# maropu/hivemall

Measured on AMD Instinct MI355X. Metric: rows/sec (node) FFM on Criteo-shaped sparse at 1/2/4/8 MI355X; logloss parity, higher is better.
Workload: dtype fp32; 1 GPU; global_batch=262144, seq_len=39, nnz_per_row=39, fields=explicit, parallelism=dp1, mix_every=10, state=fp32 V, fp32 AdaGrad accumulator per (feature, field) slot (fp32 math), state_layout=packed, reload=False, mixed_bytes_per_mix=671088656, mix_overlapped=False, mix_wire=bf16_delta, early_ramp_warmup_steps=1, linear_steps=side-table, resident_batches=8

## Files before the change

csrc/kernels/ffm.hip:

```cpp
#include <type_traits>

#include "common.h"

namespace {

struct FFMParams {
    int B, F;
    int num_features, num_fields, Kp;
    int classification;
    int train;
    int use_linear, use_bias, norm;
    int reload;
    int gstride;
    int vpad;
    int tail16;
    int gfstride;
    int sstride;
    int fstride;
    long long vfe;
    uint32_t seed;
    float eta0, eps, lambda_v;
    float alpha, beta, lambda1, lambda2;
    float min_target, max_target;
    const void* reserved;
    int32_t* defer;
    int list_mode;
    int lin_defer;
    long long lstride;
    int lpack;
    int lin_atomic;
    const int32_t* hidx;
    const int32_t* hot_id;
    float* hacc;
    int nhot;
    int hacc_on;
    float* bias_sh;
    int bias_s;
    int bias_every;
};

#define LW(p, i) ((p)[(size_t)(i) * (size_t)P.lstride])

__device__ __forceinline__ float ftrl_weight(float z, float n, float alpha, float beta,
                                             float l1, float l2) {
    if (fabsf(z) <= l1) return 0.f;
    const float s = z > 0.f ? 1.f : -1.f;
    return -(z - s * l1) / ((beta + sqrtf(n)) / alpha + l2);
}

__device__ __forceinline__ float ftrl_update(float* __restrict__ z, float* __restrict__ n,
                                             float w, float g, float alpha, float beta,
                                             float l1, float l2) {
    const float n0 = *n;
    const float n1 = n0 + g * g;
    const float sigma = (sqrtf(n1) - sqrtf(n0)) / alpha;
    const float z1 = *z + g - sigma * w;
    *z = z1;
    *n = n1;
    return ftrl_weight(z1, n1, alpha, beta, l1, l2);
}

__device__ __forceinline__ float bias_w0(const FFMParams& P, const float* bias) {
    const float z = __hip_atomic_load(bias + 1, __ATOMIC_RELAXED, __HIP_MEMORY_SCOPE_AGENT);
    const float n = __hip_atomic_load(bias + 2, __ATOMIC_RELAXED, __HIP_MEMORY_SCOPE_AGENT);
    return ftrl_weight(z, n, P.alpha, P.beta, 0.f, 0.f);
}

__device__ __forceinline__ void bias_update(const FFMParams& P, float g, float* bias) {
    const float z0 = __hip_atomic_load(bias + 1, __ATOMIC_RELAXED, __HIP_MEMORY_SCOPE_AGENT);
    const float n0 = __hip_atomic_load(bias + 2, __ATOMIC_RELAXED, __HIP_MEMORY_SCOPE_AGENT);
    const float w = ftrl_weight(z0, n0, P.alpha, P.beta, 0.f, 0.f);
    const float sigma = (sqrtf(n0 + g * g) - sqrtf(n0)) / P.alpha;
    const float dz = g - sigma * w;
    atomicAdd(bias + 1, dz);
    atomicAdd(bias + 2, g * g);
    bias[0] = ftrl_weight(z0 + dz, n0 + g * g, P.alpha, P.beta, 0.f, 0.f);
}

__device__ __forceinline__ void bias_update_sh(const FFMParams& P, float g, float z0, float n0, float* sh,
                                               float* acc) {
    const float w = ftrl_weight(z0, n0, P.alpha, P.beta, 0.f, 0.f);
    const float sigma = (sqrtf(n0 + g * g) - sqrtf(n0)) / P.alpha;
    const float dz = g - sigma * w;
    atomicAdd(sh, dz);
    atomicAdd(sh + 1, g * g);
    acc[0] += dz;
    acc[1] += g * g;
}

constexpr int HD_SIZE = 2048;
constexpr int HD12_SIZE = 1024;
constexpr int HACC_READ_STRIDE = 4;
__host__ __device__ __forceinline__ int hacc_read_off(int nhot) { return (2 * nhot + 31) & ~31; }

template <int TPB>
__device__ __forceinline__ void hacc_publish(float* __restrict__ hacc, int nhot, int tid) {
    typedef float f4v __attribute__((ext_vector_type(4)));
    float4* rd = reinterpret_cast<float4*>(hacc + hacc_read_off(nhot));
    for (int t = 2 * tid; t < nhot; t += 2 * TPB) {
        const f4v a = __builtin_nontemporal_load(reinterpret_cast<const f4v*>(hacc) + (t >> 1));
        rd[(HACC_READ_STRIDE / 4) * t] = make_float4(a.x, a.y, 0.f, 0.f);
        if (t + 1 < nhot) rd[(HACC_READ_STRIDE / 4) * (t + 1)] = make_float4(a.z, a.w, 0.f, 0.f);
    }
}
constexpr int HACC_GRID = 2048;
constexpr int HACC_GRID12 = 2304;

__device__ __forceinline__ uint32_t hash3(uint32_t a, uint32_t b, uint32_t c) {
    uint32_t h = a * 0x9E3779B1u ^ (b + 0x7F4A7C15u) * 0x85EBCA77u ^ c * 0xC2B2AE3Du;
    h ^= h >> 15; h *= 0x2C1B3C6Du; h ^= h >> 12; h *= 0x297A2D39u; h ^= h >> 15;
    return h;
}

template <bool BF>
__device__ __forceinline__ float4 ld_chunk(const void* base, size_t off) {
    if constexpr (BF) {
        const uint2 q = *reinterpret_cast<const uint2*>(reinterpret_cast<const uint16_t*>(base) + off);
        return make_float4(__uint_as_float(q.x << 16), __uint_as_float(q.x & 0xFFFF0000u),
                           __uint_as_float(q.y << 16), __uint_as_float(q.y & 0xFFFF0000u));
    } else {
        return *reinterpret_cast<const float4*>(reinterpret_cast<const float*>(base) + off);
    }
}

template <bool BF>
__device__ __forceinline__ typename std::conditional<BF, uint2, float4>::type ld_raw(const void* base, size_t off) {
    if constexpr (BF) return *reinterpret_cast<const uint2*>(reinterpret_cast<const uint16_t*>(base) + off);
    else return *reinterpret_cast<const float4*>(reinterpret_cast<const float*>(base) + off);
}

template <bool BF, typename T>
__device__ __forceinline__ float4 to_f4(const T& q) {
    if constexpr (BF) {
        return make_float4(__uint_as_float(q.x << 16), __uint_as_float(q.x & 0xFFFF0000u),
                           __uint_as_float(q.y << 16), __uint_as_float(q.y & 0xFFFF0000u));
    } else {
        return q;
    }
}

template <bool BF>
__device__ __forceinline__ void st_chunk(void* base, size_t off, float4 v, uint32_t rnd) {
    if constexpr (BF) {
        const uint32_t r2 = rnd * 0x9E3779B1u + 0x632BE5ABu;
        const uint32_t lo = hm::pack_bf16x2_sr(v.x, rnd, v.y, rnd >> 16);
        const uint32_t hi = hm::pack_bf16x2_sr(v.z, r2, v.w, r2 >> 16);
        *reinterpret_cast<uint2*>(reinterpret_cast<uint16_t*>(base) + off) = make_uint2(lo, hi);
    } else {
        *reinterpret_cast<float4*>(reinterpret_cast<float*>(base) + off) = v;
    }
}

struct SlotMeta {
    int i, f;
    float x;
};

__device__ __forceinline__ SlotMeta fetch_row_meta(const FFMParams& P, int row,
                                                   const int32_t* __restrict__ idx,
                                                   const int32_t* __restrict__ fld,
                                                   const float* __restrict__ val) {
    SlotMeta m{-1, 0, 0.f};
    const int tid = threadIdx.x;
    if (tid < P.F && row < P.B) {
        const size_t o = (size_t)row * P.F + tid;
        m.i = idx[o];
        m.f = fld ? fld[o] : tid;
        m.x = val ? val[o] : 1.f;
    }
    return m;
}

__device__ __forceinline__ float publish_row_meta(const FFMParams& P, SlotMeta m, int* s_idx,
                                                  int* s_fld, float* s_x, float* s_red) {
    const int tid = threadIdx.x;
    float sq = 0.f;
// ... 599 lines not shown
                o0 = o0 + meta * d0 * r0;
                o1 = o1 + meta * d1 * r1;
                const uint32_t h = rotl32(hrow, 5 * j + 1) ^ (0x9E3779B9u * (uint32_t)(j + 1));
                const uint4 st = make_uint4(pack_sr_hi(o0, h, rotl32(h, 16)),
                                            pack_sr_hi(o1, rotl32(h, 8), rotl32(h, 24)),
                                            pack_sr_hi(g0, rotl32(h, 4), rotl32(h, 20)),
                                            pack_sr_hi(g1, rotl32(h, 12), rotl32(h, 28)));
                if (wr >> j & 1u) *reinterpret_cast<uint4*>(vg + off[j]) = st;
            }
            if (wave == 0 && lane < F) {
                const int pi = s_m[cur][lane].x;
                if (pi >= 0) {
                    for (int f = P.num_fields; f < (int)nfld; ++f)
                        *reinterpret_cast<uint4*>(vg + ((uint32_t)pi * nfld + (uint32_t)f) * SLOT_B) = make_uint4(0u, 0u, 0u, 0u);
                }
            }
            if (mi >= 0) {
                if (P.use_linear) {
                    const float lz = s_lin[cur][1][lane];
                    const float ln = s_lin[cur][2][lane];
                    const float g = kappa * mx * scale;
                    const float n1 = ln + g * g;
                    const float z1 = lz + g - (sqrtf(n1) - sqrtf(ln)) / P.alpha * lw;
                    LW(wz, mi) = z1;
                    LW(wn, mi) = n1;
                    LW(w, mi) = ftrl_weight(z1, n1, P.alpha, P.beta, P.lambda1, P.lambda2);
                }
            }
            if (P.use_bias && tid == 0) bias_update(P, kappa, bias);
        }
        if (more) dma_lin(nxt);
    }
    __builtin_amdgcn_s_waitcnt(0x0F70);
#undef SA
#undef SB
}


typedef uint32_t u3v_t __attribute__((ext_vector_type(3)));

#define VMCNT_ENC(n) ((((n) & 15) | (((n) >> 4) << 14)) | 0x0F70)
template <bool PIN>
__device__ __forceinline__ float dot4_products_rounded(float4 c, float4 p) {
    float m0 = c.x * p.x, m1 = c.y * p.y, m2 = c.z * p.z, m3 = c.w * p.w;
    if constexpr (PIN) asm("" : "+v"(m0), "+v"(m1), "+v"(m2), "+v"(m3));
    return m0 + m1 + m2 + m3;
}

constexpr int SG32_TRAIN = 1;

template <int NS, typename OT, int TPB = 256, int ATOM = 0, int KV = 1, int KEEP = 0, int LT = 0, int CFG = 0>
__global__ __launch_bounds__(TPB) __attribute__((amdgpu_waves_per_eu(TPB / 128))) void ffm_pipe_sg32_kernel(
    FFMParams P, const int32_t* __restrict__ idx, const int32_t* __restrict__ fld,
    const float* __restrict__ val, const float* __restrict__ y, void* __restrict__ Vt,
    float* __restrict__ Gt, float* __restrict__ w, float* __restrict__ wz, float* __restrict__ wn,
    float* __restrict__ bias, float* __restrict__ pred_out, float* __restrict__ loss_out)
{
    constexpr bool SPEC = (CFG & SG32_TRAIN) != 0;
    static_assert(!SPEC || (ATOM == 0 && KV == 1 && KEEP >= 2 && sizeof(OT) == 4 && TPB % 64 == 0 &&
                            TPB >= 256 && NS <= 8 && NS * TPB < (1 << 15)),
                  "SG32_TRAIN: the default fp32 k <= 4 training launch only");
#define c_train (SPEC || P.train)
#define c_linear (SPEC || P.use_linear)
#define c_lpack (SPEC || P.lpack)
#define c_ldefer (SPEC || P.lin_defer)
#define c_bias (!SPEC && P.use_bias)
#define c_fld (SPEC || fld)
#define c_val (SPEC || val)
#define c_hacc (SPEC ? LT != 0 : P.hacc_on)
    __shared__ __attribute__((aligned(16))) float4 s_rv[NS * TPB * KV];
    __shared__ __attribute__((aligned(16))) float s_rg[NS * TPB];
    __shared__ __attribute__((aligned(16))) float4 s_t[NS * TPB * KV];
    __shared__ __attribute__((aligned(16))) int4 s_m[2][48];
    __shared__ __attribute__((aligned(16))) int s_mr[2][3][48];
    __shared__ __attribute__((aligned(16))) float s_lin[2][3][48];
    __shared__ __attribute__((aligned(16))) float4 s_lin4[2][48];
    __shared__ float s_red[TPB / 64 + 2];
    __shared__ int s_rep[TPB / 64];
    __shared__ float s_bias[4];
    __shared__ float s_bcur[2];
    __shared__ float2 s_hd[LT ? HD_SIZE : 1];
    __shared__ __attribute__((aligned(16))) float4 s_hacc[LT ? 2 : 1][48];
    __shared__ __attribute__((aligned(16))) int s_nh[LT ? 2 : 1][48];
    const int F = P.F;
    const int FF = F * F;
    const int tid = threadIdx.x, lane = tid & 63;
    const int wave = SPEC ? __builtin_amdgcn_readfirstlane(tid >> 6) : tid >> 6;
    constexpr int W_META = 1, W_LIN = 2, W_DMA = 3;
    const OT vfs = (OT)P.fstride * (16u * KV);
    const OT gfs = (OT)P.gstride * 4u;
    const int G = (int)gridDim.x;
    const int bid = (int)blockIdx.x;
    char* vb = reinterpret_cast<char*>(Vt);
    char* gb = reinterpret_cast<char*>(Gt);
    if constexpr (LT != 0) {
        for (int t = tid; t < HD_SIZE; t += TPB) s_hd[t] = make_float2(0.f, 0.f);
    }
    int nh = -1, kh = -1;
    const float* hread = LT ? P.hacc + hacc_read_off(P.nhot) : nullptr;

    int ab[NS];
    uint32_t okm = 0u;
#pragma unroll
    for (int j = 0; j < NS; ++j) {
        const int s = tid + j * TPB;
        if constexpr (SPEC) {
            const int a = s < FF ? s / F : 0, b = s < FF ? s % F : 0;
            ab[j] = (a << 4) | (b << 10) | ((s < FF ? b * F + a : s) << 16);
            okm |= (uint32_t)(s >= FF) << j | (uint32_t)(s >= FF || a == b) << (8 + j) | (uint32_t)(a < b) << (16 + j);
        } else {
            ab[j] = s < FF ? (s / F) | ((s % F) << 8) : 0;
        }
    }
#define SA(j) (SPEC ? (ab[j] >> 4) & 0x3F : ab[j] & 0xFF)
#define SB(j) (SPEC ? (ab[j] >> 10) & 0x3F : ab[j] >> 8)
#define ST(j) (SPEC ? ab[j] >> 16 : (SB(j) * F + SA(j)) * KV)

    auto dma_meta = [&](int bf, int row) {
        if (wave == W_DMA && lane < F && row < P.B) {
            const size_t o = (size_t)row * F + lane;
            __builtin_amdgcn_global_load_lds((glb_ptr_t)(idx + o), (lds_ptr_t)&s_mr[bf][0][0], 4, 0, 0);
            if (c_fld) __builtin_amdgcn_global_load_lds((glb_ptr_t)(fld + o), (lds_ptr_t)&s_mr[bf][1][0], 4, 0, 0);
            if (c_val) __builtin_amdgcn_global_load_lds((glb_ptr_t)(val + o), (lds_ptr_t)&s_mr[bf][2][0], 4, 0, 0);
        }
    };
    auto publish_meta = [&](int bf) {
        if (wave == W_META) {
            float sq = 0.f;
            if (lane < F) {
                int ri = s_mr[bf][0][lane];
                int rf = c_fld ? s_mr[bf][1][lane] : lane;
                float rx = c_val ? __int_as_float(s_mr[bf][2][lane]) : 1.f;
                if (ri < 0 || ri >= P.num_features || rf < 0 || rf >= P.num_fields) { ri = -1; rx = 0.f; rf = 0; }
                const int hb = SPEC && ri >= 0 ? (int)((uint32_t)ri * (uint32_t)vfs) : 0;
                s_m[bf][lane] = make_int4(ri, rf, __float_as_int(rx), hb);
                sq = rx * rx;
            }
            const float tot = hm::wave_sum_uniform(sq);
            if (lane == 0) s_red[TPB / 64 + bf] = (P.norm && tot > 0.f) ? rsqrtf(tot) : 1.f;
        }
    };
    auto slot = [&](int bf, int j, OT& ov, OT& og, float& xab) -> uint32_t {
        const int4 ma = s_m[bf][SA(j)], mb = s_m[bf][SB(j)];
        const bool ok = (ma.x | mb.x) >= 0 && tid + j * TPB < FF;
        const bool live = ok && SA(j) != SB(j);
        const OT i = ok ? (OT)(uint32_t)ma.x : (OT)0, f = ok ? (OT)(uint32_t)mb.y : (OT)0;
        ov = i * vfs + f * (16u * KV);
        og = i * gfs + f * 4u;
        xab = live ? __int_as_float(ma.z) * __int_as_float(mb.z) : 0.f;
        return live ? 1u : (ok ? 2u : 0u);
    };
    OT kov[KEEP ? NS : 1], kog[KEEP ? NS : 1], nov[KEEP ? NS : 1], nog[KEEP ? NS : 1];
    float kxab[KEEP ? NS : 1], nxab[KEEP ? NS : 1];
    uint32_t klive = 0u, kwr = 0u, nlive = 0u, nwr = 0u;
    int krep = 0, nrep = 0;
    auto dma_slots = [&](int bf) {
        if constexpr (KEEP) { nlive = 0u; nwr = 0u; nrep = 0; }
        if constexpr (SPEC) {
            uint32_t eq = 0u;
#pragma unroll
            for (int j = 0; j < NS; ++j) {
                const int4 ma = s_m[bf][SA(j)], mb = s_m[bf][SB(j)];
                const int both = ma.x | mb.x;
                const bool ok = (both | (int)(okm << (31 - j))) >= 0;
                const bool live = (both | (int)(okm << (23 - j))) >= 0;
                const OT ib = ok ? (OT)(uint32_t)ma.w : (OT)0, f = ok ? (OT)(uint32_t)mb.y : (OT)0;
                OT f4 = f * 4u;
                asm("" : "+v"(f4));
                nov[j] = ib + f * 16u;
                nog[j] = ib + f4;
                nxab[j] = live ? __int_as_float(ma.z) * __int_as_float(mb.z) : 0.f;
                nwr |= (uint32_t)ok << j;
                eq |= (uint32_t)(ma.x == mb.x || ma.y == mb.y) << j;
                __builtin_amdgcn_global_load_lds((glb_ptr_t)(vb + nov[j]), (lds_ptr_t)(s_rv + j * TPB + wave * 64), 16, 0, 0);
                __builtin_amdgcn_global_load_lds((glb_ptr_t)(gb + nog[j]), (lds_ptr_t)(s_rg + j * TPB + wave * 64), 4, 0, 0);
            }
            nlive = nwr & ~(okm >> 8);
            if (P.defer) nrep = (int)(eq & nwr & (okm >> 16));
            return;
        }
#pragma unroll
        for (int j = 0; j < NS; ++j) {
            OT ov, og;
            float xab;
            const uint32_t k = slot(bf, j, ov, og, xab);
            if constexpr (KEEP) {
                nov[j] = ov;
                nog[j] = og;
                nxab[j] = xab;
                nlive |= (k & 1u) << j;
                nwr |= (uint32_t)(k != 0u) << j;
                if (P.defer) nrep |= (int)slot_repeats(SA(j), SB(j), s_m[bf][SA(j)], s_m[bf][SB(j)]);
            }
#pragma unroll
            for (int q = 0; q < KV; ++q)
                __builtin_amdgcn_global_load_lds((glb_ptr_t)(vb + ov + 16u * q),
                                                 (lds_ptr_t)(s_rv + (q * NS + j) * TPB + wave * 64), 16, 0, 0);
            __builtin_amdgcn_global_load_lds((glb_ptr_t)(gb + og), (lds_ptr_t)(s_rg + j * TPB + wave * 64), 4, 0, 0);
        }
    };
    auto keep_rotate = [&]() {
        if constexpr (KEEP) {
#pragma unroll
            for (int j = 0; j < NS; ++j) { kov[j] = nov[j]; kog[j] = nog[j]; kxab[j] = nxab[j]; }
            klive = nlive; kwr = nwr; krep = nrep;
        }
    };
    const int nlin = (c_linear && c_ldefer) ? ((c_lpack || !c_train) ? 1 + (LT != 0) : 3) : 0;
    auto dma_lin = [&](int bf) {
        if (c_linear && wave == W_LIN && lane < F) {
            const int i = max(s_m[bf][lane].x, 0);
            if (c_lpack) {
                __builtin_amdgcn_global_load_lds((glb_ptr_t)&LW(w, i), (lds_ptr_t)&s_lin4[bf][0], 16, 0, 0);
                if constexpr (LT != 0)
                    __builtin_amdgcn_global_load_lds((glb_ptr_t)(hread + HACC_READ_STRIDE * max(nh, 0)), (lds_ptr_t)&s_hacc[bf][0], 16, 0, 0);
                return;
            }
            __builtin_amdgcn_global_load_lds((glb_ptr_t)&LW(w, i), (lds_ptr_t)&s_lin[bf][0][0], 4, 0, 0);
            if (c_train) {
                __builtin_amdgcn_global_load_lds((glb_ptr_t)&LW(wz, i), (lds_ptr_t)&s_lin[bf][1][0], 4, 0, 0);
                __builtin_amdgcn_global_load_lds((glb_ptr_t)&LW(wn, i), (lds_ptr_t)&s_lin[bf][2][0], 4, 0, 0);
            }
        }
    };

    int row = bid;
    if (row >= P.B) return;
    if (tid == 0) { s_bcur[0] = 0.f; s_bcur[1] = 0.f; }
    dma_meta(0, row);
    if constexpr (LT != 0) {
        if (c_hacc) hacc_publish<TPB>(P.hacc, P.nhot, tid);
    }
    __builtin_amdgcn_s_waitcnt(0x0F70);
    bar_raw();
    publish_meta(0);
    bar_raw();
    dma_slots(0);
    keep_rotate();
    if constexpr (LT != 0) {
        if (wave == W_LIN && lane < F) nh = s_m[0][lane].x >= 0 ? P.hidx[s_m[0][lane].x] : -1;
    }
    dma_lin(0);
    kh = nh;
    dma_meta(1, row + G);

    float4 fv[NS][KV];
    float fg[NS];
    OT fo[NS];
    uint32_t fwd = 0u;
    const bool bsh = c_bias && P.bias_sh;
    int bit = 0;
    float bz = 0.f, bn = 0.f;
    if (bsh && wave == W_META && lane < P.bias_s) {
        bz = __hip_atomic_load(P.bias_sh + lane * 32, __ATOMIC_RELAXED, __HIP_MEMORY_SCOPE_AGENT);
        bn = __hip_atomic_load(P.bias_sh + lane * 32 + 1, __ATOMIC_RELAXED, __HIP_MEMORY_SCOPE_AGENT);
    }
    for (int cur = 0; row < P.B; row += G, cur ^= 1) {
        const int nxt = cur ^ 1;
        const bool more = row + G < P.B;
        if constexpr (SPEC) asm volatile("" : "+v"(okm));
        if (wave == W_LIN && nlin == 3) __builtin_amdgcn_s_waitcnt(0x0F73);
        else if (wave == W_LIN && nlin == 2) __builtin_amdgcn_s_waitcnt(0x0F72);
        else if (wave == W_LIN && nlin == 1) __builtin_amdgcn_s_waitcnt(0x0F71);
        else __builtin_amdgcn_s_waitcnt(0x0F70);
        bar_raw();
        const bool bre = bsh && bit > 0 && (bit % P.bias_every) == 0;
        float nbz = bz, nbn = bn;
        if (bre && wave == W_META && lane < P.bias_s) {
            nbz = __hip_atomic_load(P.bias_sh + lane * 32, __ATOMIC_RELAXED, __HIP_MEMORY_SCOPE_AGENT);
            nbn = __hip_atomic_load(P.bias_sh + lane * 32 + 1, __ATOMIC_RELAXED, __HIP_MEMORY_SCOPE_AGENT);
        }
        if constexpr (LT != 0) {
            if (more && wave == W_LIN && lane < F) {
                const int ri = s_mr[nxt][0][lane];
                __builtin_amdgcn_global_load_lds((glb_ptr_t)(P.hidx + (ri >= 0 && ri < P.num_features ? ri : 0)),
                                                 (lds_ptr_t)&s_nh[nxt][0], 4, 0, 0);
            }
        }
        float cg[NS];
        float4 own[SPEC ? NS : 1];
#pragma unroll
        for (int j = 0; j < NS; ++j) {
            cg[j] = s_rg[j * TPB + tid];
            float4 v[KV];
#pragma unroll
            for (int q = 0; q < KV; ++q) v[q] = s_rv[(q * NS + j) * TPB + tid];
            if (fwd >> j & 1u) {
                bool same;
                if constexpr (KEEP) {
                    same = (kwr >> j & 1u) && kov[j] == fo[j];
                } else {
                    OT ov, og;
                    float xq;
                    same = slot(cur, j, ov, og, xq) != 0u && ov == fo[j];
                }
                if (same) {
#pragma unroll
                    for (int q = 0; q < KV; ++q) v[q] = fv[j][q];
                    cg[j] = fg[j];
                }
            }
            if constexpr (SPEC) {
                s_t[ST(j)] = v[0];
                own[j] = v[0];
            } else if (tid + j * TPB < FF) {
#pragma unroll
                for (int q = 0; q < KV; ++q) s_t[ST(j) + q] = v[q];
            }
        }
        fwd = 0u;
        if (more) publish_meta(nxt);
        bar_raw();
        if (more) {
            dma_slots(nxt);
            dma_meta(cur, row + 2 * G);
        }
        const float scale = s_red[TPB / 64 + cur];
        int mi = -1;
// ... 91 lines not shown
                float gs = cg[j];
#pragma unroll
                for (int q = 0; q < KV; ++q) {
                    const float4 pv = KEEP >= 2 ? kpv[j][q] : s_t[s * KV + q];
                    const float4 cv = KEEP >= 2 ? kcv[j][q] : s_t[ST(j) + q];
                    o0[q] = f2{cv.x, cv.y};
                    o1[q] = f2{cv.z, cv.w};
                    const f2 p0 = f2{pv.x, pv.y}, p1 = f2{pv.z, pv.w};
                    d0[q] = cc * p0 + ll * o0[q];
                    d1[q] = cc * p1 + ll * o1[q];
                    gs = (((gs + d0[q].x * d0[q].x) + d0[q].y * d0[q].y) + d1[q].x * d1[q].x) + d1[q].y * d1[q].y;
                }
                const float r = __builtin_amdgcn_rsqf(gs + P.eps) * -P.eta0;
                const f2 rr = {r, r};
#pragma unroll
                for (int q = 0; q < KV; ++q) {
                    const f2 n0 = o0[q] + rr * d0[q], n1 = o1[q] + rr * d1[q];
                    fv[j][q] = make_float4(n0.x, n0.y, n1.x, n1.y);
                }
                fg[j] = gs;
                fo[j] = ov;
                fwd |= 1u << j;
                if (ATOM == 1) {
                    if (live >> j & 1u) {
                        float* vp = reinterpret_cast<float*>(vb + ov);
#pragma unroll
                        for (int q = 0; q < KV; ++q) {
                            const f2 e0 = rr * d0[q], e1 = rr * d1[q];
                            atomicAdd(vp + 4 * q + 0, e0.x);
                            atomicAdd(vp + 4 * q + 1, e0.y);
                            atomicAdd(vp + 4 * q + 2, e1.x);
                            atomicAdd(vp + 4 * q + 3, e1.y);
                        }
                        atomicAdd(reinterpret_cast<float*>(gb + og), gs - cg[j]);
                    }
                    continue;
                }
#pragma unroll
                for (int q = 0; q < KV; ++q) *reinterpret_cast<float4*>(vb + ov + 16u * q) = fv[j][q];
                *reinterpret_cast<float*>(gb + og) = fg[j];
            }
            if (mi >= 0) {
                if (c_linear) {
                    const float lz = hot ? hz : (c_lpack ? s_lin4[cur][lane].y : s_lin[cur][1][lane]);
                    const float ln = hot ? hn : (c_lpack ? s_lin4[cur][lane].z : s_lin[cur][2][lane]);
                    const float g = kappa * mx * scale;
                    const float n1 = ln + g * g;
                    const float z1 = lz + g - (sqrtf(n1) - sqrtf(ln)) / P.alpha * lw;
                    const float w1 = ftrl_weight(z1, n1, P.alpha, P.beta, P.lambda1, P.lambda2);
                    if (LT && hot) {
                        const float2 d = s_hd[kh];
                        s_hd[kh] = make_float2(d.x + (g - (sqrtf(n1) - sqrtf(ln)) / P.alpha * lw), d.y + g * g);
                    } else if (ATOM == 1) {
                        atomicAdd(&LW(wz, mi), z1 - lz);
                        atomicAdd(&LW(wn, mi), g * g);
                        LW(w, mi) = w1;
                    } else if (c_lpack) {
                        *reinterpret_cast<float4*>(&LW(w, mi)) = make_float4(w1, z1, n1, s_lin4[cur][lane].w);
                    } else {
                        LW(wz, mi) = z1;
                        LW(wn, mi) = n1;
                        LW(w, mi) = w1;
                    }
                }
            }
            if (c_bias && tid == 0) {
                if (bsh) bias_update_sh(P, kappa, s_bias[1], s_bias[2], P.bias_sh + (blockIdx.x % P.bias_s) * 32, s_bcur);
                else bias_update(P, kappa, bias);
            }
        }
        if constexpr (LT != 0) {
            if (more && wave == W_LIN && lane < F) nh = s_nh[nxt][lane];
        }
        if (more) dma_lin(nxt);
        kh = nh;
        keep_rotate();
        bz = nbz;
        bn = nbn;
        ++bit;
    }
    __builtin_amdgcn_s_waitcnt(0x0F70);
    if constexpr (LT != 0) {
        bar_raw();
        if (c_hacc)
            for (int t = tid; t < 2 * P.nhot; t += TPB) {
                const float2 d = s_hd[t >> 1];
                if (d.y != 0.f || d.x != 0.f) atomicAdd(P.hacc + t, (t & 1) ? d.y : d.x);
            }
    }
#undef SA
#undef SB
#undef ST
#undef c_train
#undef c_linear
#undef c_lpack
#undef c_ldefer
#undef c_bias
#undef c_fld
#undef c_val
#undef c_hacc
}

template <int NS, typename OT, int KEEP = 0, int LT = 0>
__global__ __launch_bounds__(256) __attribute__((amdgpu_waves_per_eu(4))) void ffm_pipe_sg12_kernel(
    FFMParams P, const int32_t* __restrict__ idx, const int32_t* __restrict__ fld,
    const float* __restrict__ val, const float* __restrict__ y, void* __restrict__ Vt,
    float* __restrict__ w, float* __restrict__ wz, float* __restrict__ wn,
    float* __restrict__ bias, float* __restrict__ pred_out, float* __restrict__ loss_out)
{
    __shared__ __attribute__((aligned(16))) uint32_t s_raw[NS * 256 * 4];
    __shared__ __attribute__((aligned(16))) uint2 s_t[NS * 256];
    __shared__ __attribute__((aligned(16))) int4 s_m[2][48];
    __shared__ __attribute__((aligned(16))) int s_mr[2][3][48];
    __shared__ __attribute__((aligned(16))) float s_lin[2][3][48];
    __shared__ __attribute__((aligned(16))) float4 s_lin4[2][48];
    __shared__ float s_red[8];
    __shared__ int s_rep[4];
    __shared__ float s_bias[4];
    __shared__ float s_bcur[2];
    __shared__ float2 s_hd[LT ? HD12_SIZE : 1];
    __shared__ __attribute__((aligned(16))) float4 s_hacc[LT ? 2 : 1][48];
    __shared__ __attribute__((aligned(16))) int s_nh[LT ? 2 : 1][48];
    const int F = P.F;
    const int FF = F * F;
    const int tid = threadIdx.x, wave = tid >> 6, lane = tid & 63;
    constexpr int W_META = 1, W_LIN = 2, W_DMA = 3;
    const OT bs = (OT)P.gstride * 4u;
    const int G = gridDim.x;
    char* vb = reinterpret_cast<char*>(Vt);
    if constexpr (LT != 0) {
        for (int t = tid; t < HD12_SIZE; t += 256) s_hd[t] = make_float2(0.f, 0.f);
    }
    int nh = -1, kh = -1;
    const float* hread = LT ? P.hacc + hacc_read_off(P.nhot) : nullptr;
    const bool lin_in_tail = reinterpret_cast<const char*>(w) == vb + (size_t)P.vpad * 12;
    typedef uint32_t u3v __attribute__((ext_vector_type(3)));

    int ab[NS];
#pragma unroll
    for (int j = 0; j < NS; ++j) {
        const int s = tid + j * 256;
        ab[j] = s < FF ? (s / F) | ((s % F) << 8) : 0;
    }
#define SA(j) (ab[j] & 0xFF)
#define SB(j) (ab[j] >> 8)
    const uint32_t tid_h = (uint32_t)tid * 0x9E3779B1u;

    auto dma_meta = [&](int bf, int row) {
        if (wave == W_DMA && lane < F && row < P.B) {
            const size_t o = (size_t)row * F + lane;
            __builtin_amdgcn_global_load_lds((glb_ptr_t)(idx + o), (lds_ptr_t)&s_mr[bf][0][0], 4, 0, 0);
            if (fld) __builtin_amdgcn_global_load_lds((glb_ptr_t)(fld + o), (lds_ptr_t)&s_mr[bf][1][0], 4, 0, 0);
            if (val) __builtin_amdgcn_global_load_lds((glb_ptr_t)(val + o), (lds_ptr_t)&s_mr[bf][2][0], 4, 0, 0);
        }
    };
    auto publish_meta = [&](int bf) {
        if (wave == W_META) {
            float sq = 0.f;
            if (lane < F) {
                int ri = s_mr[bf][0][lane];
                int rf = fld ? s_mr[bf][1][lane] : lane;
                float rx = val ? __int_as_float(s_mr[bf][2][lane]) : 1.f;
                if (ri < 0 || ri >= P.num_features || rf < 0 || rf >= P.num_fields) { ri = -1; rx = 0.f; rf = 0; }
                s_m[bf][lane] = make_int4(ri, rf, __float_as_int(rx), 0);
                sq = rx * rx;
            }
            const float tot = hm::wave_sum_uniform(sq);
            if (lane == 0) s_red[4 + bf] = (P.norm && tot > 0.f) ? rsqrtf(tot) : 1.f;
        }
    };
    auto slot = [&](int bf, int j, OT& off, float& xab) -> uint32_t {
        const int4 ma = s_m[bf][SA(j)], mb = s_m[bf][SB(j)];
        const bool ok = (ma.x | mb.x) >= 0 && tid + j * 256 < FF;
        const bool live = ok && SA(j) != SB(j);
        off = ok ? (OT)(uint32_t)ma.x * bs + (OT)(uint32_t)mb.y * 12u : (OT)0;
        xab = live ? __int_as_float(ma.z) * __int_as_float(mb.z) : 0.f;
        return live ? 1u : (ok ? 2u : 0u);
    };
    OT koff[KEEP ? NS : 1], noff[KEEP ? NS : 1];
    float kxab[KEEP ? NS : 1], nxab[KEEP ? NS : 1];
    uint32_t klive = 0u, kwr = 0u, nlive = 0u, nwr = 0u;
    int krep = 0, nrep = 0;
    auto dma_slots = [&](int bf) {
        if constexpr (KEEP) { nlive = 0u; nwr = 0u; nrep = 0; }
#pragma unroll
        for (int j = 0; j < NS; ++j) {
            OT off;
            float xab;
            const uint32_t k = slot(bf, j, off, xab);
            if constexpr (KEEP) {
                noff[j] = off;
                nxab[j] = xab;
                nlive |= (k & 1u) << j;
                nwr |= (uint32_t)(k != 0u) << j;
                if (P.defer) nrep |= (int)slot_repeats(SA(j), SB(j), s_m[bf][SA(j)], s_m[bf][SB(j)]);
            }
            __builtin_amdgcn_global_load_lds((glb_ptr_t)(vb + off), (lds_ptr_t)(s_raw + (j * 256 + wave * 64) * 4),
                                             12, 0, 0);
        }
    };
    auto keep_rotate = [&]() {
        if constexpr (KEEP) {
#pragma unroll
            for (int j = 0; j < NS; ++j) { koff[j] = noff[j]; kxab[j] = nxab[j]; }
            klive = nlive; kwr = nwr; krep = nrep;
        }
    };
    auto dma_lin = [&](int bf) {
        if (P.use_linear && wave == W_LIN && lane < F) {
            const int i = s_m[bf][lane].x;
            if (i >= 0 && P.lpack) {
                __builtin_amdgcn_global_load_lds((glb_ptr_t)&LW(w, i), (lds_ptr_t)&s_lin4[bf][0], 16, 0, 0);
                if (LT && nh >= 0)
                    __builtin_amdgcn_global_load_lds((glb_ptr_t)(hread + HACC_READ_STRIDE * nh), (lds_ptr_t)&s_hacc[bf][0], 16, 0, 0);
            } else if (i >= 0) {
                __builtin_amdgcn_global_load_lds((glb_ptr_t)&LW(w, i), (lds_ptr_t)&s_lin[bf][0][0], 4, 0, 0);
                if (P.train) {
                    __builtin_amdgcn_global_load_lds((glb_ptr_t)&LW(wz, i), (lds_ptr_t)&s_lin[bf][1][0], 4, 0, 0);
                    __builtin_amdgcn_global_load_lds((glb_ptr_t)&LW(wn, i), (lds_ptr_t)&s_lin[bf][2][0], 4, 0, 0);
                }
            }
        }
    };

    int row = blockIdx.x;
    if (row >= P.B) return;
    if (tid == 0) { s_bcur[0] = 0.f; s_bcur[1] = 0.f; }
    dma_meta(0, row);
    if constexpr (LT != 0) {
        if (P.hacc_on) hacc_publish<256>(P.hacc, P.nhot, tid);
    }
    __builtin_amdgcn_s_waitcnt(0x0F70);
    bar_raw();
    publish_meta(0);
    bar_raw();
    dma_slots(0);
    keep_rotate();
    if constexpr (LT != 0) {
        if (P.hacc_on && wave == W_LIN && lane < F) nh = s_m[0][lane].x >= 0 ? P.hidx[s_m[0][lane].x] : -1;
    }
    dma_lin(0);
    kh = nh;
    dma_meta(1, row + G);

    const bool bsh = P.use_bias && P.bias_sh;
    int bit = 0;
    float bz = 0.f, bn = 0.f;
    if (bsh && wave == W_META && lane < P.bias_s) {
        bz = __hip_atomic_load(P.bias_sh + lane * 32, __ATOMIC_RELAXED, __HIP_MEMORY_SCOPE_AGENT);
        bn = __hip_atomic_load(P.bias_sh + lane * 32 + 1, __ATOMIC_RELAXED, __HIP_MEMORY_SCOPE_AGENT);
    }
    for (int cur = 0; row < P.B; row += G, cur ^= 1) {
        const int nxt = cur ^ 1;
        const bool more = row + G < P.B;
        __builtin_amdgcn_s_waitcnt(0x0F70);
        bar_raw();
        const bool bre = bsh && bit > 0 && (bit % P.bias_every) == 0;
        float nbz = bz, nbn = bn;
        if (bre && wave == W_META && lane < P.bias_s) {
            nbz = __hip_atomic_load(P.bias_sh + lane * 32, __ATOMIC_RELAXED, __HIP_MEMORY_SCOPE_AGENT);
            nbn = __hip_atomic_load(P.bias_sh + lane * 32 + 1, __ATOMIC_RELAXED, __HIP_MEMORY_SCOPE_AGENT);
        }
        if constexpr (LT != 0) {
            if (P.hacc_on && more && wave == W_LIN && lane < F) {
                const int ri = s_mr[nxt][0][lane];
                __builtin_amdgcn_global_load_lds((glb_ptr_t)(P.hidx + (ri >= 0 && ri < P.num_features ? ri : 0)),
                                                 (lds_ptr_t)&s_nh[nxt][0], 4, 0, 0);
            }
        }
        float cg[NS];
#pragma unroll
        for (int j = 0; j < NS; ++j) {
            const uint4 q = *reinterpret_cast<const uint4*>(s_raw + (j * 256 + tid) * 4);
            asm volatile("" :: "v"(q.w));
            cg[j] = __uint_as_float(q.z);
            if (tid + j * 256 < FF) s_t[SB(j) * F + SA(j)] = make_uint2(q.x, q.y);
        }
        if (more) publish_meta(nxt);
        bar_raw();
        if (more) {
            dma_slots(nxt);
            dma_meta(cur, row + 2 * G);
        }
        if constexpr (LT != 0) {
            if (P.hacc_on && more && wave == W_LIN) {
                __builtin_amdgcn_s_waitcnt(VMCNT_ENC(NS));
                if (lane < F) nh = s_nh[nxt][lane];
            }
        }
        const float scale = s_red[4 + cur];
        int mi = -1;
        float mx = 0.f, lw = 0.f;
        int hot = 0;
        float hz = 0.f, hn = 0.f;
        if (wave == W_LIN && lane < F) {
            const int4 m = s_m[cur][lane];
            mi = m.x;
            mx = __int_as_float(m.z);
            lw = P.lpack ? s_lin4[cur][lane].x : s_lin[cur][0][lane];
            if constexpr (LT != 0) {
                if (P.hacc_on && mi >= 0 && kh >= 0) {
                    const float4 a = s_hacc[cur][lane];
                    const float2 d = s_hd[kh];
                    hz = a.x + d.x;
                    hn = a.y + d.y;
                    hot = 1;
                    lw = hn > 0.f ? ftrl_weight(hz, hn, P.alpha, P.beta, P.lambda1, P.lambda2) : lw;
                }
            }
        }
        uint32_t live = 0u, wr = 0u;
        float xab[NS];
        uint2 kpv[KEEP >= 2 ? NS : 1], kcv[KEEP >= 2 ? NS : 1];
        float part = 0.f;
        int rep = 0;
        if constexpr (KEEP) { live = klive; wr = kwr; rep = krep; }
#pragma unroll
// ... 32 lines not shown
        if (P.train && rdup && P.defer) {
            defer_row(P, row);
        } else if (P.train) {
            const float ks = kappa * scale * scale;
            uint32_t hrow = (P.seed ^ ((uint32_t)row * 0x85EBCA77u)) + tid_h;
            hrow ^= hrow >> 16;
            hrow *= 0x7FEB352Du;
            hrow ^= hrow >> 15;
#pragma unroll
            for (int j = 0; j < NS; ++j) {
                if (!(wr >> j & 1u)) continue;
                OT off;
                if constexpr (KEEP) {
                    off = koff[j];
                } else {
                    float xj;
                    slot(cur, j, off, xj);
                }
                const int s = tid + j * 256;
                const uint2 pv = KEEP >= 2 ? kpv[j] : s_t[s];
                const uint2 cv = KEEP >= 2 ? kcv[j] : s_t[SB(j) * F + SA(j)];
                const float c = ks * xab[j];
                const float lj = (live >> j & 1u) ? P.lambda_v : 0.f;
                const f2 cc = {c, c}, ll = {lj, lj};
                f2 o0 = bf2_to_f2(cv.x), o1 = bf2_to_f2(cv.y);
                const f2 p0 = bf2_to_f2(pv.x), p1 = bf2_to_f2(pv.y);
                const f2 d0 = cc * p0 + ll * o0, d1 = cc * p1 + ll * o1;
                const float gs = (((cg[j] + d0.x * d0.x) + d0.y * d0.y) + d1.x * d1.x) + d1.y * d1.y;
                const float r = __builtin_amdgcn_rsqf(gs + P.eps) * -P.eta0;
                const f2 rr = {r, r};
                o0 = o0 + rr * d0;
                o1 = o1 + rr * d1;
                const uint32_t h = rotl32(hrow, 5 * j + 1) ^ (0x9E3779B9u * (uint32_t)(j + 1));
                *reinterpret_cast<u3v*>(vb + off) = u3v{pack_sr_hi(o0, h, rotl32(h, 16)),
                                                        pack_sr_hi(o1, rotl32(h, 8), rotl32(h, 24)),
                                                        __float_as_uint(gs)};
            }
            {
                const int npad = P.vpad - P.num_fields;
                const int per = npad + P.tail16;
                for (int q = tid; q < F * per; q += 256) {
                    const int a = q / per, kk = q - a * per;
                    const int i = s_m[cur][a].x;
                    if (i < 0) continue;
                    char* blk = vb + (OT)(uint32_t)i * bs;
                    if (kk < npad) *reinterpret_cast<u3v*>(blk + (P.num_fields + kk) * 12) = u3v{0u, 0u, 0u};
                    else if (!(lin_in_tail && kk == npad))
                        *reinterpret_cast<uint4*>(blk + P.vpad * 12 + 16 * (kk - npad)) = make_uint4(0u, 0u, 0u, 0u);
                }
            }
            if (mi >= 0 && P.use_linear) {
                const float lz = hot ? hz : (P.lpack ? s_lin4[cur][lane].y : s_lin[cur][1][lane]);
                const float ln = hot ? hn : (P.lpack ? s_lin4[cur][lane].z : s_lin[cur][2][lane]);
                const float g = kappa * mx * scale;
                const float n1 = ln + g * g;
                const float z1 = lz + g - (sqrtf(n1) - sqrtf(ln)) / P.alpha * lw;
                const float w1 = ftrl_weight(z1, n1, P.alpha, P.beta, P.lambda1, P.lambda2);
                if (LT && hot) {
                    const float2 d = s_hd[kh];
                    s_hd[kh] = make_float2(d.x + (g - (sqrtf(n1) - sqrtf(ln)) / P.alpha * lw), d.y + g * g);
                } else if (P.lpack) {
                    *reinterpret_cast<float4*>(&LW(w, mi)) = make_float4(w1, z1, n1, 0.f);
                } else {
                    LW(wz, mi) = z1;
                    LW(wn, mi) = n1;
                    LW(w, mi) = w1;
                }
            }
            if (P.use_bias && tid == 0) {
                if (bsh) bias_update_sh(P, kappa, s_bias[1], s_bias[2], P.bias_sh + (blockIdx.x % P.bias_s) * 32, s_bcur);
                else bias_update(P, kappa, bias);
            }
        }
        if (more) dma_lin(nxt);
        kh = nh;
        keep_rotate();
        bz = nbz;
        bn = nbn;
        ++bit;
    }
    __builtin_amdgcn_s_waitcnt(0x0F70);
    if constexpr (LT != 0) {
        bar_raw();
        if (P.hacc_on)
            for (int t = tid; t < 2 * P.nhot; t += 256) {
                const float2 d = s_hd[t >> 1];
                if (d.y != 0.f || d.x != 0.f) atomicAdd(P.hacc + t, (t & 1) ? d.y : d.x);
            }
    }
#undef SA
#undef SB
}


int default_blocks(int B, int grid, int cap = 256 * 8 * 4) {
    return grid > 0 ? grid : (B < cap ? B : cap);
}

struct FFMArgs {
    const int32_t *idx, *fld;
    const float *val, *y;
    void *V, *G;
    float *w, *wz, *wn, *bias, *pred, *loss;
};

using KernelV = void (*)(FFMParams, const int32_t*, const int32_t*, const float*, const float*, void*,
                         float*, float*, float*, float*, float*, float*);
template <typename GT>
using KernelVG = void (*)(FFMParams, const int32_t*, const int32_t*, const float*, const float*, void*, GT*,
                          float*, float*, float*, float*, float*, float*);

void launch(KernelV k, int blocks, int tpb, size_t lds, hipStream_t stream, const FFMParams& P, const FFMArgs& a) {
    hipLaunchKernelGGL(k, dim3(blocks), dim3(tpb), lds, stream, P, a.idx, a.fld, a.val, a.y, a.V, a.w, a.wz, a.wn,
                       a.bias, a.pred, a.loss);
}
template <typename GT>
void launch(KernelVG<GT> k, int blocks, int tpb, size_t lds, hipStream_t stream, const FFMParams& P, const FFMArgs& a) {
    hipLaunchKernelGGL(k, dim3(blocks), dim3(tpb), lds, stream, P, a.idx, a.fld, a.val, a.y, a.V,
                       reinterpret_cast<GT*>(a.G), a.w, a.wz, a.wn, a.bias, a.pred, a.loss);
}

template <int N0, int... NR, typename Fn>
void with_ns(int need, Fn&& f) {
    if constexpr (sizeof...(NR) == 0) f(std::integral_constant<int, N0>{});
    else if (need <= N0) f(std::integral_constant<int, N0>{});
    else with_ns<NR...>(need, f);
}

template <bool BF>
int dispatch_lean(const FFMParams& P, const FFMArgs& a, int grid, hipStream_t stream) {
    const size_t slot_b = BF ? 16 : 32;
    if (P.Kp != 4 || P.F > 45) return -1;
    if ((size_t)P.num_features * (size_t)P.fstride * slot_b >= ((size_t)1 << 32)) return -1;
    const size_t lean_lds = (size_t)P.F * P.F * 16 + (size_t)P.F * 16 + 16 * 4;
    const int need = (P.F * P.F + 255) / 256;
    const int blocks = default_blocks(P.B, grid);
    if (blocks <= 0) return 0;
    with_ns<2, 4, 6, 8>(need, [&](auto ns) {
        constexpr int NS = decltype(ns)::value;
        if constexpr (BF) launch(ffm_pipe_kernel<NS>, blocks, 256, 0, stream, P, a);
        else launch(ffm_lean_kernel<NS>, blocks, 256, lean_lds, stream, P, a);
    });
    HM_LAUNCH_RET();
}

__global__ __launch_bounds__(256) void ffm_hacc_kernel(FFMParams P, float* __restrict__ w, int dir) {
    const int h = blockIdx.x * 256 + threadIdx.x;
    if (h >= P.nhot) return;
    float4* rp = reinterpret_cast<float4*>(&LW(w, P.hot_id[h]));
    float2* ap = reinterpret_cast<float2*>(P.hacc) + h;
    const float4 r = *rp;
    if (dir == 0) {
        *ap = make_float2(r.y, r.z);
        *reinterpret_cast<float4*>(P.hacc + hacc_read_off(P.nhot) + HACC_READ_STRIDE * h) = make_float4(r.y, r.z, 0.f, 0.f);
    } else {
        const float2 a = *ap;
        const float nw = a.y > 0.f ? ftrl_weight(a.x, a.y, P.alpha, P.beta, P.lambda1, P.lambda2) : r.x;
        *rp = make_float4(nw, a.x, a.y, r.w);
    }
}

template <typename Fn>
int with_side_table(const FFMParams& Q, float* w, hipStream_t stream, Fn&& train) {
    if (Q.hacc_on) {
        hipLaunchKernelGGL(ffm_hacc_kernel, dim3((Q.nhot + 255) / 256), dim3(256), 0, stream, Q, w, 0);
        HM_LAUNCH_RET_IF_ERR();
    }
    train();
    if (Q.hacc_on) {
        HM_LAUNCH_RET_IF_ERR();
        hipLaunchKernelGGL(ffm_hacc_kernel, dim3((Q.nhot + 255) / 256), dim3(256), 0, stream, Q, w, 1);
    }
    HM_LAUNCH_RET();
}

int dispatch_sg12(const FFMParams& P, const FFMArgs& a, int grid, hipStream_t stream) {
    if (P.Kp != 4 || P.F > 45) return -1;
    const bool wide = (size_t)P.num_features * (size_t)P.gstride * 4 >= ((size_t)1 << 32);
    const int need = (P.F * P.F + 255) / 256;
    int blocks = default_blocks(P.B, grid, 256 * 8 * 8);
    if (blocks <= 0) return 0;
    FFMParams Q = P;
    Q.hacc_on = P.lin_atomic == 4 && P.lin_defer && P.nhot <= HD12_SIZE && blocks > 1 && !wide;
    if (Q.hacc_on && grid <= 0) blocks = default_blocks(P.B, grid, HACC_GRID12);
    return with_side_table(Q, a.w, stream, [&] {
        with_ns<2, 4, 6, 8>(need, [&](auto ns) {
            constexpr int NS = decltype(ns)::value;
            if (wide) launch(ffm_pipe_sg12_kernel<NS, uint64_t>, blocks, 256, 0, stream, Q, a);
            else if (Q.hacc_on) launch(ffm_pipe_sg12_kernel<NS, uint32_t, 2, 1>, blocks, 256, 0, stream, Q, a);
            else launch(ffm_pipe_sg12_kernel<NS, uint32_t, 2>, blocks, 256, 0, stream, Q, a);
        });
    });
}

constexpr int SG32_TRAIN_TPB = 512;

template <int TPB, int CFG>
void launch_sg32_train(const FFMParams& Q, const FFMArgs& a, int blocks, hipStream_t stream) {
    const int need = (Q.F * Q.F + TPB - 1) / TPB;
    auto go = [&](auto ns) {
        constexpr int NS = decltype(ns)::value;
        if (Q.hacc_on) launch(ffm_pipe_sg32_kernel<NS, uint32_t, TPB, 0, 1, 2, 1, CFG>, blocks, TPB, 0, stream, Q, a);
        else launch(ffm_pipe_sg32_kernel<NS, uint32_t, TPB, 0, 1, 2, 0, CFG>, blocks, TPB, 0, stream, Q, a);
    };
    static_assert(TPB == 256 || TPB == 512, "a slot-count ladder for this TPB");
    if constexpr (TPB == 512) with_ns<2, 3, 4>(need, go);
    else with_ns<2, 4, 6, 8>(need, go);
}

int dispatch_sg32(const FFMParams& P, const FFMArgs& a, int grid, int variant, hipStream_t stream) {
    if ((P.Kp != 4 && P.Kp != 8) || P.F > 45 || P.vpad <= 0) return -1;
    const bool wide = (size_t)P.num_features * (size_t)P.fstride * (size_t)(P.Kp * 4) >= ((size_t)1 << 32) ||
                      (size_t)P.num_features * (size_t)P.gstride * 4 >= ((size_t)1 << 32);
    const int tpb = P.Kp == 8 ? 512 : 256;
    const int need = (P.F * P.F + tpb - 1) / tpb;
    int blocks = default_blocks(P.B, grid);
    if (blocks <= 0) return 0;
    FFMParams Q = P;
    Q.hacc_on = P.lin_atomic == 4 && P.lin_defer && blocks > 1 && !wide && variant != 6;
    if (Q.hacc_on && grid <= 0) blocks = default_blocks(P.B, grid, HACC_GRID);
    if (P.Kp == 8)
        return with_side_table(Q, a.w, stream, [&] {
            with_ns<2, 3, 4>(need, [&](auto ns) {
                constexpr int NS = decltype(ns)::value;
                if (wide) launch(ffm_pipe_sg32_kernel<NS, uint64_t, 512, 0, 2>, blocks, 512, 0, stream, Q, a);
                else if (Q.hacc_on) launch(ffm_pipe_sg32_kernel<NS, uint32_t, 512, 0, 2, 1, 1>, blocks, 512, 0, stream, Q, a);
                else if (variant == 6) launch(ffm_pipe_sg32_kernel<NS, uint32_t, 512, 1, 2>, blocks, 512, 0, stream, Q, a);
                else launch(ffm_pipe_sg32_kernel<NS, uint32_t, 512, 0, 2, 1>, blocks, 512, 0, stream, Q, a);
            });
        });
// ... 169 lines not shown
```

hivemall_amd/ops/ffm.py:

```python
from __future__ import annotations

import ctypes
import os
from dataclasses import dataclass

import numpy as np
import torch

from .. import _native


@dataclass
class FFMHyper:
    eta0: float = 0.2
    eps: float = 1.0
    lambda_v: float = 1e-4
    alpha: float = 0.2
    beta: float = 1.0
    lambda1: float = 1e-3
    lambda2: float = 1e-4
    min_target: float = -3.4e38
    max_target: float = 3.4e38
    classification: bool = True
    use_linear: bool = True
# ... 77 lines not shown
               and wz.data_ptr() == w.data_ptr() + 4 and wn.data_ptr() == w.data_ptr() + 8
               and w.data_ptr() % 16 == 0 and ls % 4 == 0
               and os.environ.get("HM_FFM_LPACK", "1") != "0")
    if not pack:
        assert ls == 1 or w.is_cuda, "CPU FFM state: contiguous linear tables"
    return ls, pack


def linear_mix_tensors(state: dict) -> list:
    w = state["w"]
    ls, pack = _lin_addressing(state)
    if pack:
        return [torch.as_strided(w, (w.shape[0], 4), (ls, 1))]
    return [state["wz"], state["wn"], w]


def new_state_tables(num_features: int, num_fields: int, kp: int, dtype, device,
                     packed: bool, slot_g: bool = False) -> tuple[torch.Tensor, torch.Tensor]:
    if slot_g:
        if packed and dtype == torch.bfloat16 and kp == 4:
            fs, bs = slot12_layout(num_fields)
            buf = torch.zeros((num_features, bs), dtype=torch.uint8, device=device)
            sl = buf[:, :fs * 12]
            V = sl.view(torch.bfloat16).view(num_features, fs, 6)[:, :num_fields, :4]
            G = sl.view(torch.float32).view(num_features, fs, 3)[:, :num_fields, 2]
            return V, G
        if packed:
            fs, bs, goff = slot_block_layout(num_fields, kp, dtype)
            es = torch.empty(0, dtype=dtype).element_size()
            buf = torch.zeros((num_features, bs), dtype=torch.uint8, device=device)
            V = buf[:, :goff].view(dtype).view(num_features, fs, kp)[:, :num_fields]
            G = buf[:, goff:goff + fs * 4].view(torch.float32)[:, :num_fields]
            assert V.stride(0) * es == bs and G.stride(0) * 4 == bs
            return V, G
        return (torch.zeros((num_features, num_fields, kp), dtype=dtype, device=device),
                torch.zeros((num_features, num_fields), dtype=torch.float32, device=device))
    if packed:
        fs = padded_fields(num_fields, kp, dtype)
        VG = torch.zeros((num_features, fs, 2, kp), dtype=dtype, device=device)
        return VG[:, :num_fields, 0, :], VG[:, :num_fields, 1, :]
    shape = (num_features, num_fields, kp)
    return (torch.zeros(shape, dtype=dtype, device=device),
            torch.zeros(shape, dtype=dtype, device=device))


_DEFER: dict = {}
BIAS_SHARDS = int(os.environ.get("HM_FFM_BIAS_SHARDS", "64"))
BIAS_EVERY = int(os.environ.get("HM_FFM_BIAS_EVERY", "32"))
_BIAS_SH: dict = {}


def _launch_key(device: torch.device):
    return (device, _native.stream_of(device))


def _bias_shards(device: torch.device) -> torch.Tensor:
    key = _launch_key(device)
    sh = _BIAS_SH.get(key)
    if sh is None or sh.shape[0] != BIAS_SHARDS:
        sh = torch.zeros((BIAS_SHARDS, 32), dtype=torch.float32, device=device)
        _BIAS_SH[key] = sh
    return sh
_DEFER_ON = os.environ.get("HM_FFM_DEFER", "1") != "0"
_LIN_DEFER = int(os.environ.get("HM_FFM_LIN_DEFER", "1") != "0")
LIN_MODES = (0, 4)
_LIN_ATOMIC = int(os.environ.get("HM_FFM_LIN_ATOMIC", "4"))
_LIN_HOT_N = min(int(os.environ.get("HM_FFM_LIN_HOT", "2048")), 2048)
_LIN_HOT: dict = {}
_LIN_HOT_KEEP = 8


_LIN_HOT_REFRESH = int(os.environ.get("HM_FFM_LIN_HOT_REFRESH", "256"))


def _hacc_read_off(nhot: int) -> int:
    return (2 * nhot + 31) & ~31


def _hacc_views(hacc: torch.Tensor, nhot: int):
    off = _hacc_read_off(nhot)
    return hacc[:2 * nhot].view(nhot, 2), hacc[off:off + 4 * nhot].view(nhot, 4)


def _lin_hot_tables(state: dict, idx: torch.Tensor, nhot: int):
    w = state["w"]
    nf = w.shape[0]
    key = (w.device, w.data_ptr(), nf, nhot)
    t = _LIN_HOT.get(key)
    if t is not None:
        t[3][0] += 1
        if _LIN_HOT_REFRESH > 0 and t[3][0] % _LIN_HOT_REFRESH == 0:
            del _LIN_HOT[key]
            t = None
    if t is None:
        cnt = torch.bincount(idx.reshape(-1).long().clamp(0, nf - 1), minlength=nf)
        top = torch.argsort(cnt, descending=True)[:nhot]
        top = top[cnt[top] > 0].to(torch.int32)
        hidx = torch.full((nf,), -1, dtype=torch.int32, device=w.device)
        hidx[top.long()] = torch.arange(top.numel(), dtype=torch.int32, device=w.device)
        n = max(1, top.numel())
        hacc = torch.zeros(_hacc_read_off(n) + 4 * n, dtype=torch.float32, device=w.device)
        while len(_LIN_HOT) >= _LIN_HOT_KEEP:
            _LIN_HOT.pop(next(iter(_LIN_HOT)))
        t = _LIN_HOT[key] = (hidx, top, hacc, [0])
    return t[:3]


def _defer_buffer(device: torch.device, B: int) -> torch.Tensor:
    key = _launch_key(device)
    buf = _DEFER.get(key)
    if buf is None or buf.numel() < 1 + B:
        buf = torch.empty(1 + max(B, 1 << 16), dtype=torch.int32, device=device)
        _DEFER[key] = buf
    return buf


def _has_multihot(idx: torch.Tensor, fld: torch.Tensor | None) -> bool:
    if idx.numel() == 0 or idx.shape[1] < 2:
        return False
    big = torch.iinfo(torch.int32).max
    pos = torch.arange(idx.shape[1], device=idx.device, dtype=torch.int32)

    def rep(t: torch.Tensor, valid: torch.Tensor) -> bool:
        u = torch.where(valid, t, big - pos.unsqueeze(0))
        s = u.sort(dim=1).values
        return bool((s[:, 1:] == s[:, :-1]).any().item())

    valid = idx >= 0
    if rep(idx, valid):
        return True
    return fld is not None and rep(fld, valid & (fld >= 0))


def ffm_step(state: dict, idx: torch.Tensor, fld: torch.Tensor | None, val: torch.Tensor | None,
             y: torch.Tensor | None, hyper: FFMHyper, train: bool = True,
             pred: torch.Tensor | None = None, loss: torch.Tensor | None = None,
             grid: int = 0, variant: int | None = None, lin_mode: int | None = None) -> None:
    auto = variant is None and _VARIANT == 0
    variant = _VARIANT if variant is None else int(variant)
    lin_mode = _LIN_ATOMIC if lin_mode is None else int(lin_mode)
    for what, v, live in (("kernel variant", variant, VARIANTS), ("linear mode", lin_mode, LIN_MODES)):
        if v not in live:
            raise ValueError(f"FFM {what} {v}: the live values are {live}")
    V = state["V"]
    B, F = idx.shape
    NF, NFLD, Kp = V.shape
    assert idx.dtype == torch.int32 and idx.is_contiguous()
    for t in (fld, val, y, pred, loss):
        if t is not None:
            assert t.device == V.device and t.is_contiguous(), "tensor device/layout mismatch"
    if fld is not None:
        assert fld.dtype == torch.int32 and fld.shape == idx.shape
    if val is not None:
        assert val.dtype == torch.float32 and val.shape == idx.shape
    if y is not None:
        assert y.shape[0] == B
    if pred is not None:
        assert pred.shape[0] >= B
    if loss is not None:
        assert loss.shape[0] >= B
    if V.is_cuda and train and int(grid) == 1 and auto and _has_multihot(idx, fld):
        variant = 1
    G = state["G"]
    bf16 = V.dtype == torch.bfloat16
    slot_g = G.dim() == 2
    gstride = 0
    block = (0, 0)
    if slot_g:
        assert G.dtype == torch.float32 and G.shape == V.shape[:2] and G.stride(1) in (1, 3), \
            "per-slot G: fp32 [num_features, num_fields], field stride 1 (or 3: 12-B bf16 slots)"
        assert V.stride(2) == 1 and (V.stride(1) == Kp or (G.stride(1) == 3 and V.stride(1) == 6)), \
            "V: [NF, FS, Kp] slots (or the V part of 12-B {V | G} slots)"
        packed = False
        gstride = G.stride(0)
        es = V.element_size()
        d = G.data_ptr() - V.data_ptr()
        bs = V.stride(0) * es
        if G.stride(1) == 3:
            fs, bs12 = slot12_layout(NFLD)
            assert V.is_cuda and bf16 and d == 8 and G.stride(0) * 4 == bs12, "12-B slot layout"
            block = (fs, (bs12 - fs * 12) // 16)
        elif V.is_cuda and G.stride(1) == 1 and 0 < d < bs and d % (Kp * es) == 0 and G.stride(0) * 4 == bs:
            vpad = d // (Kp * es)
            tail = bs - d - vpad * 4
# ... 47 lines not shown
```

Measured before the change: 92.56 million rows/s.

## Gate hot-accumulator republish with per-XCC flush counters instead of every block

Previously every block republished the whole hot linear-accumulator table into the strided read copy at kernel start. A small control region now sits after the read copy, holding a global flush counter, per-XCC last-seen counters and a publish interval (default 64, set from the host). Thread 0 of each block checks whether enough flushes have happened since its XCC last published, and only then does the block republish. This removes most of the redundant per-block global traffic at kernel start. The cost is that readers may see a read copy that is staler by up to the interval, which could affect logloss parity, and the gate check uses relaxed atomics, so two blocks may race and both publish.

```diff
diff --git a/csrc/kernels/ffm.hip b/csrc/kernels/ffm.hip
--- a/csrc/kernels/ffm.hip
+++ b/csrc/kernels/ffm.hip
@@ -92,6 +92,27 @@
 constexpr int HD12_SIZE = 1024;
 constexpr int HACC_READ_STRIDE = 4;
 __host__ __device__ __forceinline__ int hacc_read_off(int nhot) { return (2 * nhot + 31) & ~31; }
+__host__ __device__ __forceinline__ int hacc_ctl_off(int nhot) { return (hacc_read_off(nhot) + 4 * nhot + 31) & ~31; }
+constexpr int HACC_CTL_LINE = 32;
+constexpr int HACC_CTL_SEEN = 1, HACC_CTL_EVERY = 9, HACC_CTL_LINES = 10;
+
+struct HaccGate { uint32_t flushed, seen, every; int x; };
+__device__ __forceinline__ HaccGate hacc_gate_load(float* __restrict__ hacc, int nhot) {
+    uint32_t* ctl = reinterpret_cast<uint32_t*>(hacc + hacc_ctl_off(nhot));
+    HaccGate g;
+    g.x = (int)(__builtin_amdgcn_s_getreg(20 | (0 << 6) | (3 << 11)) & 7u);
+    g.flushed = __hip_atomic_load(ctl, __ATOMIC_RELAXED, __HIP_MEMORY_SCOPE_AGENT);
+    g.seen = __hip_atomic_load(ctl + HACC_CTL_LINE * (HACC_CTL_SEEN + g.x), __ATOMIC_RELAXED, __HIP_MEMORY_SCOPE_AGENT);
+    g.every = __hip_atomic_load(ctl + HACC_CTL_LINE * HACC_CTL_EVERY, __ATOMIC_RELAXED, __HIP_MEMORY_SCOPE_AGENT);
+    return g;
+}
+__device__ __forceinline__ bool hacc_gate_open(const HaccGate& g) { return g.flushed - g.seen >= g.every; }
+__device__ __forceinline__ void hacc_gate_mark(float* __restrict__ hacc, int nhot, const HaccGate& g) {
+    reinterpret_cast<uint32_t*>(hacc + hacc_ctl_off(nhot))[HACC_CTL_LINE * (HACC_CTL_SEEN + g.x)] = g.flushed;
+}
+__device__ __forceinline__ void hacc_count_flush(float* __restrict__ hacc, int nhot) {
+    __hip_atomic_fetch_add(reinterpret_cast<uint32_t*>(hacc + hacc_ctl_off(nhot)), 1u, __ATOMIC_RELAXED, __HIP_MEMORY_SCOPE_AGENT);
+}
 
 template <int TPB>
 __device__ __forceinline__ void hacc_publish(float* __restrict__ hacc, int nhot, int tid) {
@@ -857,6 +878,7 @@
     __shared__ float2 s_hd[LT ? HD_SIZE : 1];
     __shared__ __attribute__((aligned(16))) float4 s_hacc[LT ? 2 : 1][48];
     __shared__ __attribute__((aligned(16))) int s_nh[LT ? 2 : 1][48];
+    __shared__ int s_pub;
     const int F = P.F;
     const int FF = F * F;
     const int tid = threadIdx.x, lane = tid & 63;
@@ -1003,12 +1025,26 @@
     if (row >= P.B) return;
     if (tid == 0) { s_bcur[0] = 0.f; s_bcur[1] = 0.f; }
     dma_meta(0, row);
+    HaccGate gate = {0u, 0u, 0u, 0};
     if constexpr (LT != 0) {
-        if (c_hacc) hacc_publish<TPB>(P.hacc, P.nhot, tid);
+        if (c_hacc && tid == 0) gate = hacc_gate_load(P.hacc, P.nhot);
     }
     __builtin_amdgcn_s_waitcnt(0x0F70);
+    if constexpr (LT != 0) {
+        if (c_hacc && tid == 0) {
+            const bool open = hacc_gate_open(gate);
+            s_pub = open;
+            if (open) hacc_gate_mark(P.hacc, P.nhot, gate);
+        }
+    }
     bar_raw();
     publish_meta(0);
+    if constexpr (LT != 0) {
+        if (c_hacc && __builtin_amdgcn_readfirstlane(s_pub)) {
+            hacc_publish<TPB>(P.hacc, P.nhot, tid);
+            __builtin_amdgcn_s_waitcnt(0x0F70);
+        }
+    }
     bar_raw();
     dma_slots(0);
     keep_rotate();
@@ -1266,11 +1302,13 @@
     __builtin_amdgcn_s_waitcnt(0x0F70);
     if constexpr (LT != 0) {
         bar_raw();
-        if (c_hacc)
+        if (c_hacc) {
             for (int t = tid; t < 2 * P.nhot; t += TPB) {
                 const float2 d = s_hd[t >> 1];
                 if (d.y != 0.f || d.x != 0.f) atomicAdd(P.hacc + t, (t & 1) ? d.y : d.x);
             }
+            if (tid == 0) hacc_count_flush(P.hacc, P.nhot);
+        }
     }
 #undef SA
 #undef SB
@@ -1305,6 +1343,7 @@
     __shared__ float2 s_hd[LT ? HD12_SIZE : 1];
     __shared__ __attribute__((aligned(16))) float4 s_hacc[LT ? 2 : 1][48];
     __shared__ __attribute__((aligned(16))) int s_nh[LT ? 2 : 1][48];
+    __shared__ int s_pub;
     const int F = P.F;
     const int FF = F * F;
     const int tid = threadIdx.x, wave = tid >> 6, lane = tid & 63;
@@ -1411,12 +1450,26 @@
     if (row >= P.B) return;
     if (tid == 0) { s_bcur[0] = 0.f; s_bcur[1] = 0.f; }
     dma_meta(0, row);
+    HaccGate gate = {0u, 0u, 0u, 0};
     if constexpr (LT != 0) {
-        if (P.hacc_on) hacc_publish<256>(P.hacc, P.nhot, tid);
+        if (P.hacc_on && tid == 0) gate = hacc_gate_load(P.hacc, P.nhot);
     }
     __builtin_amdgcn_s_waitcnt(0x0F70);
+    if constexpr (LT != 0) {
+        if (P.hacc_on && tid == 0) {
+            const bool open = hacc_gate_open(gate);
+            s_pub = open;
+            if (open) hacc_gate_mark(P.hacc, P.nhot, gate);
+        }
+    }
     bar_raw();
     publish_meta(0);
+    if constexpr (LT != 0) {
+        if (P.hacc_on && __builtin_amdgcn_readfirstlane(s_pub)) {
+            hacc_publish<256>(P.hacc, P.nhot, tid);
+            __builtin_amdgcn_s_waitcnt(0x0F70);
+        }
+    }
     bar_raw();
     dma_slots(0);
     keep_rotate();
@@ -1615,11 +1668,13 @@
     __builtin_amdgcn_s_waitcnt(0x0F70);
     if constexpr (LT != 0) {
         bar_raw();
-        if (P.hacc_on)
+        if (P.hacc_on) {
             for (int t = tid; t < 2 * P.nhot; t += 256) {
                 const float2 d = s_hd[t >> 1];
                 if (d.y != 0.f || d.x != 0.f) atomicAdd(P.hacc + t, (t & 1) ? d.y : d.x);
             }
+            if (tid == 0) hacc_count_flush(P.hacc, P.nhot);
+        }
     }
 #undef SA
 #undef SB
@@ -1679,6 +1734,7 @@
 
 __global__ __launch_bounds__(256) void ffm_hacc_kernel(FFMParams P, float* __restrict__ w, int dir) {
     const int h = blockIdx.x * 256 + threadIdx.x;
+    if (dir == 0 && h <= 8) reinterpret_cast<uint32_t*>(P.hacc + hacc_ctl_off(P.nhot))[HACC_CTL_LINE * h] = 0u;
     if (h >= P.nhot) return;
     float4* rp = reinterpret_cast<float4*>(&LW(w, P.hot_id[h]));
     float2* ap = reinterpret_cast<float2*>(P.hacc) + h;
diff --git a/hivemall_amd/ops/ffm.py b/hivemall_amd/ops/ffm.py
--- a/hivemall_amd/ops/ffm.py
+++ b/hivemall_amd/ops/ffm.py
@@ -183,6 +183,21 @@
     return hacc[:2 * nhot].view(nhot, 2), hacc[off:off + 4 * nhot].view(nhot, 4)
 
 
+HACC_PUBLISH_EVERY = int(os.environ.get("HM_FFM_HACC_EVERY", "64"))
+_HACC_CTL_LINE = 32
+_HACC_CTL_LINES = 10
+
+
+def _hacc_ctl_off(nhot: int) -> int:
+    return (_hacc_read_off(nhot) + 4 * nhot + 31) & ~31
+
+
+def _hacc_ctl(hacc: torch.Tensor, nhot: int):
+    off = _hacc_ctl_off(nhot)
+    c = hacc[off:off + _HACC_CTL_LINE * _HACC_CTL_LINES].view(torch.int32).view(_HACC_CTL_LINES, _HACC_CTL_LINE)[:, 0]
+    return c[0:1], c[1:9], c[9:10]
+
+
 def _lin_hot_tables(state: dict, idx: torch.Tensor, nhot: int):
     w = state["w"]
     nf = w.shape[0]
@@ -200,7 +215,8 @@
         hidx = torch.full((nf,), -1, dtype=torch.int32, device=w.device)
         hidx[top.long()] = torch.arange(top.numel(), dtype=torch.int32, device=w.device)
         n = max(1, top.numel())
-        hacc = torch.zeros(_hacc_read_off(n) + 4 * n, dtype=torch.float32, device=w.device)
+        hacc = torch.zeros(_hacc_ctl_off(n) + _HACC_CTL_LINE * _HACC_CTL_LINES, dtype=torch.float32, device=w.device)
+        _hacc_ctl(hacc, n)[2].fill_(HACC_PUBLISH_EVERY)
         while len(_LIN_HOT) >= _LIN_HOT_KEEP:
             _LIN_HOT.pop(next(iter(_LIN_HOT)))
         t = _LIN_HOT[key] = (hidx, top, hacc, [0])
```

Result: faster. 94.48 million rows/s, median of 6 (+2.1%).
